# DixianZhu/deBWT

Measured on NVIDIA B200. Metric: bwt_build_throughput, higher is better.
Workload: dtype u64

## Files before the change

### debwt_b200/api.py

```python
from __future__ import annotations

import ctypes
from typing import Sequence

import numpy as np

from . import binding
from .binding import DebwtError, ShardStats, Stats, c_p, c_u64, check, lib


def _ptr(a: np.ndarray):
    return a.ctypes.data_as(c_p)


def join_records(records: Sequence) -> tuple[np.ndarray, np.ndarray]:
    arrs = [np.frombuffer(r.encode() if isinstance(r, str) else bytes(r), dtype=np.uint8)
            if not isinstance(r, np.ndarray) else r.astype(np.uint8, copy=False) for r in records]
    if not arrs:
        raise DebwtError("no records")
    n = sum(a.size for a in arrs) + len(arrs)
    text = np.empty(n, dtype=np.uint8)
    seps = np.empty(len(arrs), dtype=np.uint64)
    pos = 0
    for i, a in enumerate(arrs):
# ... 132 lines not shown
    def locate(self, patterns: Sequence) -> tuple[np.ndarray, np.ndarray]:
        pats = [p.encode() if isinstance(p, str) else bytes(p) for p in patterns]
        offs = np.zeros(len(pats) + 1, dtype=np.uint64)
        offs[1:] = np.cumsum([len(p) for p in pats])
        blob = np.frombuffer(b"".join(pats) + b"\0", dtype=np.uint8)
        hits = np.zeros(len(pats) + 1, dtype=np.uint64)
        check(lib().debwt_index_locate(self._h, _ptr(blob), _ptr(offs), len(pats), _ptr(hits), c_p(0), 0))
        pos = np.empty(int(hits[-1]), dtype=np.uint64)
        if pos.size:
            check(lib().debwt_index_locate(self._h, _ptr(blob), _ptr(offs), len(pats), _ptr(hits), _ptr(pos), pos.size))
        return hits, pos

    def verify(self, text=None, device_ptr: int | None = None, n_symbols: int | None = None):
        bad, ms = c_u64(), ctypes.c_float()
        if device_ptr is not None:
            check(lib().debwt_verify_text_device(self._h, c_p(device_ptr), n_symbols, ctypes.byref(bad), ctypes.byref(ms)))
        else:
            text = np.ascontiguousarray(text, dtype=np.uint8)
            check(lib().debwt_verify_text(self._h, _ptr(text), text.size, ctypes.byref(bad), ctypes.byref(ms)))
        return int(bad.value), float(ms.value)

    def stats(self) -> dict:
        s = Stats()
        check(lib().debwt_get_stats(self._h, ctypes.byref(s)))
        return s.as_dict()


def build_bwt(records: Sequence, device: int = 0, k: int = 32):
    with BwtBuilder(device) as b:
        b.set_records(records)
        b.build(k)
        return b.result()


def write_outputs(path: str, words: np.ndarray, sharp: np.ndarray, dollar: np.ndarray):
    words.astype("<u8", copy=False).tofile(path)
    sharp.astype("<u8", copy=False).tofile(path + ".#")
    dollar.astype("<u8", copy=False).tofile(path + ".$")


def read_outputs(path: str, n_symbols: int):
    words = np.fromfile(path, dtype="<u8").astype(np.uint64, copy=False)
    if words.size != (n_symbols + 31) // 32:
        raise DebwtError(f"{path}: {words.size} words, but {n_symbols} symbols need {(n_symbols + 31) // 32}")
    sharp = np.fromfile(path + ".#", dtype="<u8").astype(np.uint64, copy=False)
    dollar = np.fromfile(path + ".$", dtype="<u8").astype(np.uint64, copy=False)
    if dollar.size != 1:
        raise DebwtError(f"{path}.$: {dollar.size} values, expected 1")
    return words, sharp, dollar


def record_offsets(positions, seps) -> tuple[np.ndarray, np.ndarray]:
    pos = np.asarray(positions, dtype=np.uint64)
    seps = np.asarray(seps, dtype=np.uint64)
    if pos.size and int(pos.max()) > int(seps[-1]):
        raise ValueError(f"position {int(pos.max())} is beyond the text ({int(seps[-1]) + 1} symbols)")
    rec = np.searchsorted(seps, pos, side="left")
    starts = np.concatenate(([0], seps[:-1] + 1)).astype(np.uint64)
    return rec.astype(np.int64), pos - starts[rec]


def k_pack(text: np.ndarray, device: int = 0) -> np.ndarray:
    text = np.ascontiguousarray(text, dtype=np.uint8)
    out = np.empty((text.size + 32 + 31) // 32, dtype=np.uint64)
    check(lib().debwt_k_pack(device, _ptr(text), text.size, _ptr(out)))
    return out


def k_extract(text: np.ndarray, seps: np.ndarray, device: int = 0) -> np.ndarray:
    text = np.ascontiguousarray(text, dtype=np.uint8)
    seps = np.ascontiguousarray(seps, dtype=np.uint64)
    out = np.empty(text.size - 32 * seps.size, dtype=np.uint64)
    check(lib().debwt_k_extract(device, _ptr(text), text.size, _ptr(seps), seps.size, _ptr(out)))
    return out


def k_radix_sort(keys: np.ndarray, device: int = 0, cfg: int = 0):
    k = np.ascontiguousarray(keys, dtype=np.uint64).copy()
    ms = ctypes.c_float()
    check(lib().debwt_k_radix_sort_u64(device, _ptr(k), k.size, cfg, ctypes.byref(ms)))
    return k, ms.value


def k_rle(sorted_keys: np.ndarray, device: int = 0):
    s = np.ascontiguousarray(sorted_keys, dtype=np.uint64)
    km = np.empty(s.size, dtype=np.uint64)
    ct = np.empty(s.size, dtype=np.uint64)
    d = c_u64()
    check(lib().debwt_k_rle(device, _ptr(s), s.size, _ptr(km), _ptr(ct), ctypes.byref(d)))
    return km[:d.value].copy(), ct[:d.value].copy()


def k_group_masks(text: np.ndarray, seps: np.ndarray, device: int = 0) -> np.ndarray:
    text = np.ascontiguousarray(text, dtype=np.uint8)
    seps = np.ascontiguousarray(seps, dtype=np.uint64)
    out = np.empty(text.size - 32 * seps.size, dtype=np.uint16)
    check(lib().debwt_k_group_masks(device, _ptr(text), text.size, _ptr(seps), seps.size, _ptr(out)))
    return out


def bench_sort(n: int, device: int = 0, cfg: int = 0, iters: int = 5) -> float:
    ms = ctypes.c_float()
    check(lib().debwt_bench_sort(device, n, cfg, iters, ctypes.byref(ms)))
    return ms.value


def bench_sort_passes(n: int, device: int = 0, cfg: int = 0, iters: int = 5):
    ms, msp = ctypes.c_float(), ctypes.c_float()
    check(lib().debwt_bench_sort_passes(device, n, cfg, iters, ctypes.byref(ms), ctypes.byref(msp)))
    return ms.value, msp.value


def verify_bwt_device(bwt_ptr: int, n_symbols: int, sharp_rows: np.ndarray, dollar_row: int, text_ptr: int, device: int = 0):
    sharp = np.ascontiguousarray(sharp_rows, dtype=np.uint64)
    bad, ms = c_u64(), ctypes.c_float()
    check(lib().debwt_verify_bwt_device(device, c_p(bwt_ptr), n_symbols, _ptr(sharp), sharp.size, int(dollar_row), c_p(text_ptr),
                                        ctypes.byref(bad), ctypes.byref(ms)))
    return int(bad.value), float(ms.value)


def k_codes(text: np.ndarray, seps: np.ndarray, device: int = 0):
    text = np.ascontiguousarray(text, dtype=np.uint8)
    seps = np.ascontiguousarray(seps, dtype=np.uint64)
    cap = text.size + 64
    codes = np.empty(cap, dtype=np.uint8)
    head, spi, prev = np.empty(cap, dtype=np.uint64), np.empty(cap, dtype=np.uint64), np.empty(cap, dtype=np.uint8)
    nc, nb = c_u64(), c_u64()
    check(lib().debwt_k_codes(device, _ptr(text), text.size, _ptr(seps), seps.size, _ptr(codes), cap, ctypes.byref(nc), _ptr(head),
                              _ptr(spi), _ptr(prev), cap, ctypes.byref(nb)))
    return codes[:nc.value].copy(), head[:nb.value].copy(), spi[:nb.value].copy(), prev[:nb.value].copy()


def k_sort_blue(codes: np.ndarray, seg_offsets: np.ndarray, spindex: np.ndarray, prev: np.ndarray, device: int = 0):
    codes = np.ascontiguousarray(codes, dtype=np.uint8)
    offs = np.ascontiguousarray(seg_offsets, dtype=np.uint64)
    spi = np.ascontiguousarray(spindex, dtype=np.uint64).copy()
    prv = np.ascontiguousarray(prev, dtype=np.uint8).copy()
    check(lib().debwt_k_sort_blue(device, _ptr(codes), codes.size, _ptr(offs), offs.size - 1, _ptr(spi), _ptr(prv)))
    return spi, prv


def verify_walk_device(bwt_ptr: int, n_symbols: int, sharp_rows: np.ndarray, dollar_row: int, tail_ptr: int, steps: int, device: int = 0):
    sharp = np.ascontiguousarray(sharp_rows, dtype=np.uint64)
    bad = c_u64()
    carr = np.zeros(6, dtype=np.uint64)
    check(lib().debwt_verify_walk_device(device, c_p(bwt_ptr), n_symbols, _ptr(sharp), sharp.size, int(dollar_row), c_p(tail_ptr), steps,
                                         ctypes.byref(bad), _ptr(carr)))
    return int(bad.value), carr


class Shard:

    def __init__(self, device: int, rank: int, world: int, group_tag: str, same_process: bool = False, sort_config: int = 0):
        self._h = c_p()
        self.rank, self.world, self.device = rank, world, device
        check(lib().debwt_shard_create(ctypes.byref(self._h), device, rank, world, group_tag.encode(), int(same_process)))
        if sort_config:
            lib().debwt_shard_set_sort_config(self._h, sort_config)

    def close(self):
        if self._h:
            lib().debwt_shard_destroy(self._h)
            self._h = c_p()

    def __enter__(self):
        return self
# ... 59 lines not shown
```

### debwt_b200/build.py

```python
from __future__ import annotations

import concurrent.futures as cf
import os
import shutil
import subprocess

HERE = os.path.dirname(os.path.abspath(__file__))
CSRC = os.path.join(HERE, "csrc")
OBJ = os.path.join(HERE, "_build")
LIB = os.path.join(HERE, "libdebwt_b200.so")
SOURCES = ["radix_sort.cu", "radix_sort_tma.cu", "stages.cu", "bluesort.cu", "dist_kernels.cu", "dev_api.cu", "api.cu", "index.cu", "synth.cu", "shard.cu"]
HEADERS = ["common.cuh", "radix_sort.cuh", "radix_common.cuh", "ctx.cuh", "shmcomm.h", "stages.cuh", "stages_dev.cuh", "special.cuh", "dist_kernels.cuh",
           os.path.join("..", "..", "include", "debwt_b200.h"), os.path.join("..", "..", "include", "debwt_b200_dev.h")]
NVCC_FLAGS = ["-gencode", "arch=compute_100a,code=sm_100a", "-lineinfo", "-O3", "-std=c++17",
              "-Xcompiler", "-fPIC", "-Xcompiler", "-O2"]


def _nvcc() -> str:
    for cand in (shutil.which("nvcc"), "/usr/local/cuda/bin/nvcc"):
        if cand and os.path.isfile(cand):
            return cand
    raise RuntimeError("nvcc not found")


def _stale(target: str, deps) -> bool:
    if not os.path.isfile(target):
        return True
    t = os.path.getmtime(target)
    return any(os.path.getmtime(d) > t for d in deps)


def build(force: bool = False, verbose: bool = False) -> str:
    os.makedirs(OBJ, exist_ok=True)
    nvcc = _nvcc()
    hdrs = [os.path.join(CSRC, h) for h in HEADERS]
    jobs = []
    for src in SOURCES:
        s = os.path.join(CSRC, src)
        o = os.path.join(OBJ, src.replace(".cu", ".o"))
        if force or _stale(o, [s] + hdrs):
            jobs.append([nvcc] + NVCC_FLAGS + ["-c", s, "-o", o])
    if jobs:
        with cf.ThreadPoolExecutor(max_workers=len(jobs)) as ex:
            for cmd, res in zip(jobs, ex.map(lambda c: subprocess.run(c, capture_output=True, text=True), jobs)):
                if verbose or res.returncode:
                    print(" ".join(cmd))
                    print(res.stdout + res.stderr)
                if res.returncode:
                    raise RuntimeError("nvcc failed: " + " ".join(cmd))
    objs = [os.path.join(OBJ, s.replace(".cu", ".o")) for s in SOURCES]
    if force or jobs or _stale(LIB, objs):
        cmd = [nvcc, "-shared", "-o", LIB] + objs + ["-gencode", "arch=compute_100a,code=sm_100a", "-lcudart", "-lrt", "-lpthread"]
        res = subprocess.run(cmd, capture_output=True, text=True)
        if res.returncode:
            print(res.stdout + res.stderr)
            raise RuntimeError("link failed")
    return LIB


if __name__ == "__main__":
    print(build(verbose=True))
```

### debwt_b200/csrc/api.cu

```cuda
#include <algorithm>
#include <cstring>
#include <map>
#include <mutex>
#include <string>
#include <tuple>
#include <vector>

#include "../../include/debwt_b200.h"
#include "../../include/debwt_b200_dev.h"
#include "radix_sort.cuh"
#include "stages.cuh"
#include "special.cuh"
#include "ctx.cuh"
#include "dist_kernels.cuh"

namespace debwt {

static thread_local std::string g_err;
unsigned g_launches = 0;
unsigned long long g_launches_total = 0;
void set_error(const std::string& msg) { g_err = msg; }

#define FAIL(msg)            \
    do {                     \
        debwt::set_error(msg); \
        return -1;           \
    } while (0)

template <typename T>
static int dalloc(DevPool& pool, T** p, size_t count) { return pool.alloc(reinterpret_cast<void**>(p), count * sizeof(T)); }

struct Special {
    u64 pos;
    u32 j;
    u32 rec;
    u64 ins, row;
    u64 w0, w1;
    u8 chr, next;
    bool emit;
};



int build_special_tables(const SpecialInfo* info, const u64* seps, u64 R, std::vector<u64>& ins, std::vector<u64>& rows,
                         std::vector<u8>& chr, std::vector<u64>& emit_pos, std::vector<u64>& tail_pos) {
    const u64 nspec = 32 * R;
    std::vector<Special> sp(nspec);
    std::vector<char> seen_rank(nspec, 0);
    for (u64 t = 0; t < nspec; ++t) {
        const SpecialInfo& o = info[t];
        if (o.rank >= nspec || seen_rank[o.rank]) FAIL("internal: special suffix ranks are not a permutation");
        seen_rank[o.rank] = 1;
        Special& x = sp[o.rank];
        x.pos = seps[t >> 5] - (t & 31); x.j = (u32)(t & 31); x.rec = (u32)(t >> 5); x.emit = false;
        x.ins = o.ins; x.chr = o.prev; x.w0 = o.w0; x.w1 = o.w1; x.next = o.next;
    }
    ins.resize(nspec); rows.resize(nspec); chr.resize(nspec); tail_pos.assign(R, 0); emit_pos.clear();
    for (u64 t = 0; t < nspec; ++t) {
        ins[t] = sp[t].ins;
        if (t && ins[t] < ins[t - 1]) FAIL("internal: special insertion points are not monotone");
        rows[t] = ins[t] + t;
        chr[t] = sp[t].chr;
    }
    std::map<std::tuple<u32, u64, u64>, std::vector<u64>> groups;
    for (u64 t = 0; t < nspec; ++t) {
        const u32 j = sp[t].j;
        if (j == 31) { sp[t].emit = true; tail_pos[sp[t].rec] = sp[t].pos; continue; }
        if (sp[t].rec + 1 == R) continue;
        const u64 before = j ? (sp[t].w0 & ~(~0ull >> (2 * j))) : 0;
        const u64 after = sp[t].w1 & ~(~0ull >> (2 * (30 - j)));
        groups[std::make_tuple(j, before, j == 30 ? 0 : after)].push_back(t);
    }
    for (auto& g : groups) {
        if (g.second.size() < 2) continue;
        u32 seen = 0;
        for (u64 t : g.second) seen |= 1u << sp[t].next;
        if (seen & (seen - 1))
            for (u64 t : g.second) sp[t].emit = true;
    }
    for (u64 t = 0; t < nspec; ++t) if (sp[t].emit) emit_pos.push_back(sp[t].pos);
    return 0;
}

}

using namespace debwt;

namespace {

std::mutex g_pool_mutex;

int bind_device(int device) {
// ... 154 lines not shown

int debwt_set_text(debwt_ctx* c, const char* text, uint64_t n, const uint64_t* seps, uint64_t n_records) {
    if (!c || !text || !seps) FAIL("null argument");
    if (bind_device(c->device)) return -1;
    reset_input(c);
    if (check_seps(seps, n_records, n)) return -1;
    c->seps.assign(seps, seps + n_records);
    c->n = n; c->n_rec = n_records;
    c->pool.hint(n * 19 + (320ull << 20));
    CUDA_TRY(cudaEventRecord(c->ev[0], c->st));
    if (dalloc(c->pool, &c->d_ascii, n + 64)) return -1;
    CUDA_TRY(cudaMemcpyAsync(c->d_ascii, text, n, cudaMemcpyHostToDevice, c->st));
    CUDA_TRY(cudaEventRecord(c->ev[1], c->st));
    CUDA_TRY(cudaStreamSynchronize(c->st));
    CUDA_TRY(cudaEventElapsedTime(&c->stats.ms_h2d, c->ev[0], c->ev[1]));
    c->input_mark = c->pool.mark();
    return 0;
}

int debwt_set_text_device(debwt_ctx* c, const void* d_text, uint64_t n, const uint64_t* seps, uint64_t n_records) {
    if (!c || !d_text || !seps) FAIL("null argument");
    if (bind_device(c->device)) return -1;
    reset_input(c);
    if (check_seps(seps, n_records, n)) return -1;
    if (reinterpret_cast<uintptr_t>(d_text) & 15) FAIL("device text must be 16-byte aligned");
    c->seps.assign(seps, seps + n_records);
    c->n = n; c->n_rec = n_records;
    c->pool.hint(n * 18 + (320ull << 20));
    c->d_ascii_ext = reinterpret_cast<const u8*>(d_text);
    c->input_mark = c->pool.mark();
    return 0;
}

int debwt_build(debwt_ctx* c, int k) {
    if (!c) FAIL("null context");
    if (k < 12 || k > 32) FAIL("-k: k-mer length (from 12 to 32, default 32)");
    if (c->loaded) FAIL("the context holds a loaded result (debwt_set_result), not an input: set an input before building");
    if (c->n == 0) FAIL("no input set");
    if (bind_device(c->device)) return -1;
    const u8* ascii = c->d_ascii_ext ? c->d_ascii_ext : c->d_ascii;
    if (c->ing.active) FAIL("streaming input is still open: call debwt_ingest_end first");
    if (!ascii && !c->d_packed) FAIL("input was consumed by a previous build; set it again");
    cudaStream_t st = c->st;
    DevPool& pool = c->pool;
    pool.rewind(c->input_mark);
    drop_index(c);
    c->built = false;
    const u64 n = c->n, R = c->n_rec, nk = n - 32 * R;
    debwt_stats& S = c->stats;
    const float keep_h2d = S.ms_h2d;
    S = debwt_stats{};
    S.ms_h2d = keep_h2d;
    S.n_symbols = n; S.n_records = R; S.n_keys = nk; S.n_special = 32 * R;
    g_launches = 0;
    int evi = 0;
    auto mark = [&]() { cudaEventRecord(c->ev[evi++], st); };
    mark();

    u64* d_seps = nullptr; u64* d_text = nullptr; u32* d_err = nullptr;
    if (dalloc(pool, &d_seps, R)) return -1;
    CUDA_TRY(cudaMemcpyAsync(d_seps, c->seps.data(), R * 8, cudaMemcpyHostToDevice, st));
    if (c->d_packed) {
        d_text = c->d_packed;
        d_err = c->d_packed_err;
    } else {
        if (dalloc(pool, &d_text, text_words(n)) || dalloc(pool, &d_err, 4)) return -1;
        CUDA_TRY(cudaMemsetAsync(d_err, 0, 16, st));
        PackPolicy pol;
        pol.resolve = c->resolve_ambiguous; pol.seed = c->ambiguity_seed;
        if (k_pack(ascii, n, d_text, d_err, st, pol)) return -1;
        if (c->d_ascii) { pool.adopt(c->d_ascii, n + 64); c->d_ascii = nullptr; }
    }
    mark();

    u64 *d_ka = nullptr, *d_kb = nullptr;
    if (dalloc(pool, &d_ka, nk + 2) || dalloc(pool, &d_kb, nk + 2)) return -1;
    if (k_extract(d_text, n, d_seps, R, d_ka, st)) return -1;
    mark();

    void* d_sortws = nullptr;
    if (pool.alloc(&d_sortws, sort_workspace_bytes(nk, c->sort_cfg))) return -1;
    SortWorkspace ws;
    sort_workspace_bind(ws, d_sortws, nk, c->sort_cfg);
    int sweeps = 0;
    ws.ev_sweep_begin = c->ev[11]; ws.ev_sweep_end = c->ev[12]; ws.sweeps_out = &sweeps;
    const unsigned launches_before_sort = g_launches;
    u64* d_keys = nullptr;
    KeyIndex ki;
    ki.bits = key_index_bits(nk);
    if (dalloc(pool, &ki.idx, (1ull << ki.bits) + 2) || k_key_index_init(ki, st)) return -1;
    bool index_marked = false;
    ws.key_index = ki.idx; ws.key_index_bits = ki.bits; ws.key_index_done = &index_marked;
    const bool text_hist = text_digit_hist_applies(n, R);
    if (text_hist && (radix_sort_clear(ws, st) || k_text_digit_hist(d_text, n, d_seps, R, ws.hist, st))) return -1;
    if (radix_sort_u64(d_ka, d_kb, nk, ws, st, &d_keys, text_hist)) return -1;
    S.sort_launches = g_launches - launches_before_sort;
    S.sort_sweeps = (u32)sweeps;
    pool.adopt(d_keys == d_ka ? d_kb : d_ka, (nk + 2) * 8);
    pool.adopt(d_sortws, sort_workspace_bytes(nk, c->sort_cfg));
    u32 h_err[2] = {0, 0};
    CUDA_TRY(cudaMemcpyAsync(h_err, d_err, 8, cudaMemcpyDeviceToHost, st));
    mark();

    u16* d_gmask = nullptr;
    if (dalloc(pool, &d_gmask, nk + 2)) return -1;
    CUDA_TRY(cudaMemsetAsync(d_gmask, 0, (nk + 2) * 2, st));
    if (k_key_index_finish(d_keys, nk, ki, index_marked, st)) return -1;
    if (k_mark_edges(d_keys, nk, ki, d_gmask, st)) return -1;
    if (k_mark_heads_tails(d_text, d_seps, R, d_keys, nk, ki, d_gmask, st)) return -1;
    void* d_brws = nullptr; u64* d_tot = nullptr;
    if (pool.alloc(&d_brws, branch_workspace_bytes(nk)) || dalloc(pool, &d_tot, 4)) return -1;
    if (k_branch_count(d_keys, nk, d_gmask, true, d_brws, d_tot, st)) return -1;
    u64 h_tot[2] = {0, 0};
    CUDA_TRY(cudaMemcpyAsync(h_tot, d_tot, 16, cudaMemcpyDeviceToHost, st));
    CUDA_TRY(cudaStreamSynchronize(st));
    if (h_err[0]) FAIL(c->resolve_ambiguous ? "input contains a symbol that is neither a base nor an IUPAC ambiguity code"
                                            : "input contains a symbol other than A, C, G, T (either case)");
    if (h_err[1] != R) FAIL("input contains '#' or '$' inside a record (they are reserved for the record separators)");
    BranchTable bt;
    bt.n_branch = h_tot[0]; bt.n_blue = h_tot[1];
    S.n_branch = bt.n_branch; S.n_blue = bt.n_blue;
    {
        int bits = 8;
        while (bits < 27 && (1ull << bits) < 2 * bt.n_branch) ++bits;
        bt.bits = bits;
    }
    if (dalloc(pool, &bt.kmer, bt.n_branch + 1) || dalloc(pool, &bt.head, bt.n_branch + 1) ||
        dalloc(pool, &bt.blue, bt.n_branch + 2) || dalloc(pool, &bt.cursor, bt.n_branch + 1) ||
        dalloc(pool, &bt.bidx, BranchTable::index_words(bt.bits)))
        return -1;
    CUDA_TRY(cudaMemsetAsync(bt.cursor, 0, (bt.n_branch + 1) * 4, st));
    if (k_branch_write(d_keys, nk, d_gmask, d_brws, bt, st)) return -1;
    {
        const u32 m32 = (u32)bt.n_blue;
        CUDA_TRY(cudaMemcpyAsync(bt.blue + bt.n_branch, &m32, 4, cudaMemcpyHostToDevice, st));
    }
    if (k_branch_index(bt, st)) return -1;
    int id_bits = 1;
    while (id_bits < 64 && (bt.n_branch >> id_bits)) ++id_bits;
    const bool group_by_sort = id_bits <= 28 && n < (1ull << 32) && bt.n_blue > 1 &&
                               c->blue_grouping == 2;
    bt.hbits = BranchTable::hash_bits(bt.n_branch);
    bt.hmode = group_by_sort ? 0 : 1;
    if (dalloc(pool, &bt.hslots, 1ull << bt.hbits) || k_branch_hash(bt, st)) return -1;
    mark();

    const u64 nspec = 32 * R;
    std::vector<SpecialInfo> info(nspec);
    std::vector<u64> h_ins(nspec);
    u64* d_ins = nullptr;
    if (dalloc(pool, &d_ins, nspec)) return -1;
    {
        SpecialInfo* d_info = nullptr;
        if (dalloc(pool, &d_info, nspec)) return -1;
        if (k_special_scan(d_text, d_seps, R, d_keys, nk, ki, d_info, st)) return -1;
        CUDA_TRY(cudaMemcpyAsync(info.data(), d_info, nspec * sizeof(SpecialInfo), cudaMemcpyDeviceToHost, st));
        CUDA_TRY(cudaStreamSynchronize(st));
    }
    std::vector<u64> h_rows, h_emit_pos, h_tail_pos;
    std::vector<u8> h_chr;
    if (build_special_tables(info.data(), c->seps.data(), R, h_ins, h_rows, h_chr, h_emit_pos, h_tail_pos)) return -1;
    u64 *d_rows = nullptr, *d_emit = nullptr, *d_tail = nullptr, *d_tail_idx = nullptr;
    u8* d_chr = nullptr;
    if (dalloc(pool, &d_rows, nspec) || dalloc(pool, &d_chr, nspec) || dalloc(pool, &d_emit, h_emit_pos.size() + 1) ||
        dalloc(pool, &d_tail, R) || dalloc(pool, &d_tail_idx, R))
        return -1;
    CUDA_TRY(cudaMemcpyAsync(d_rows, h_rows.data(), nspec * 8, cudaMemcpyHostToDevice, st));
    CUDA_TRY(cudaMemcpyAsync(d_chr, h_chr.data(), nspec, cudaMemcpyHostToDevice, st));
    CUDA_TRY(cudaMemcpyAsync(d_ins, h_ins.data(), nspec * 8, cudaMemcpyHostToDevice, st));
    CUDA_TRY(cudaMemcpyAsync(d_emit, h_emit_pos.data(), h_emit_pos.size() * 8, cudaMemcpyHostToDevice, st));
    CUDA_TRY(cudaMemcpyAsync(d_tail, h_tail_pos.data(), R * 8, cudaMemcpyHostToDevice, st));
    mark();

    const u64 nbw = (n + 31) / 32;
    u32 *d_mo = nullptr, *d_wp = nullptr;
    u64* d_blue = nullptr;
    void* d_scanws = nullptr;
    const int id_shift = 64 - id_bits;
    u64 *d_bka = nullptr, *d_bkb = nullptr, *d_bcount = nullptr;
    void* d_bsortws = nullptr;
    const int bcfg = kDefaultSortCfg;
    if (dalloc(pool, &d_mo, nbw + 2) || dalloc(pool, &d_wp, nbw + 2) || pool.alloc(&d_scanws, scan_workspace_bytes(nbw)))
// ... 562 lines not shown
```

### debwt_b200/csrc/dev_api.cu

```cuda
#include <string.h>

#include <vector>

#include "../../include/debwt_b200_dev.h"
#include "dist_kernels.cuh"
#include "radix_sort.cuh"
#include "special.cuh"

using namespace debwt;

namespace {
inline cudaStream_t S(void* s) { return reinterpret_cast<cudaStream_t>(s); }
inline KeyIndex KI(const void* idx, int bits) {
    KeyIndex k;
    k.idx = reinterpret_cast<u32*>(const_cast<void*>(idx));
    k.bits = bits;
    return k;
}
inline BranchTable BT(const void* kmer, const void* head, const void* blue, void* cursor, const void* bidx, int bits,
                      u64 nb, u64 nblue) {
    BranchTable b;
    b.n_branch = nb; b.n_blue = nblue;
    b.kmer = reinterpret_cast<u64*>(const_cast<void*>(kmer));
    b.head = reinterpret_cast<u32*>(const_cast<void*>(head));
    b.blue = reinterpret_cast<u32*>(const_cast<void*>(blue));
    b.cursor = reinterpret_cast<u32*>(cursor);
    b.bidx = reinterpret_cast<u32*>(const_cast<void*>(bidx));
    b.bits = bits;
    return b;
}
#define P64(x) reinterpret_cast<u64*>(const_cast<void*>(static_cast<const void*>(x)))
#define P32(x) reinterpret_cast<u32*>(const_cast<void*>(static_cast<const void*>(x)))
#define P16(x) reinterpret_cast<u16*>(const_cast<void*>(static_cast<const void*>(x)))
#define P8(x) reinterpret_cast<u8*>(const_cast<void*>(static_cast<const void*>(x)))
}

extern "C" {

int debwt_dev_init(int device) {
    CUDA_TRY(cudaSetDevice(device));
    cudaMemPool_t mp;
    CUDA_TRY(cudaDeviceGetDefaultMemPool(&mp, device));
    unsigned long long thr = ~0ull;
    CUDA_TRY(cudaMemPoolSetAttribute(mp, cudaMemPoolAttrReleaseThreshold, &thr));
    return 0;
}

int debwt_dev_pack(const void* d_ascii, uint64_t n, void* d_words, uint64_t nwords, void* d_err, void* stream) {
    return k_pack_words(P8(d_ascii), n, P64(d_words), nwords, P32(d_err), S(stream));
}

int debwt_dev_extract(const void* d_words, uint64_t pos_lo, uint64_t pos_hi, const void* d_seps, uint64_t n_rec,
                      uint64_t idx_base, void* d_keys, void* stream) {
    return k_extract_range(P64(d_words), pos_lo, pos_hi, P64(d_seps), n_rec, idx_base, P64(d_keys), S(stream));
}

int debwt_dev_extract_slice(const void* d_words, uint64_t n_symbols, uint64_t pos_lo, uint64_t pos_hi, const void* d_seps,
                            uint64_t n_rec, uint64_t idx_base, void* d_keys, void* stream) {
    return k_extract_slice(P64(d_words), n_symbols, pos_lo, pos_hi, P64(d_seps), n_rec, idx_base, P64(d_keys), S(stream));
}

uint64_t debwt_dev_sort_workspace_bytes(uint64_t n, int cfg) { return sort_workspace_bytes(n, cfg); }
uint64_t debwt_dev_branch_workspace_bytes(uint64_t n) { return branch_workspace_bytes(n) + 64; }
uint64_t debwt_dev_scan_workspace_bytes(uint64_t n_words) { return scan_workspace_bytes(n_words) + 64; }

int debwt_dev_sort(void* d_a, void* d_b, uint64_t n, int cfg, void* d_workspace, int* result_in_b, void* stream) {
    SortWorkspace ws;
    sort_workspace_bind(ws, d_workspace, n, cfg);
    u64* res = nullptr;
    if (radix_sort_u64(P64(d_a), P64(d_b), n, ws, S(stream), &res)) return -1;
    if (result_in_b) *result_in_b = (res == P64(d_b)) ? 1 : 0;
    return 0;
}

int debwt_dev_sort_timed(void* d_a, void* d_b, uint64_t n, int cfg, void* d_workspace, int* result_in_b, float* ms_total,
                         float* ms_sweeps, int* n_sweeps, void* stream) {
    cudaStream_t st = S(stream);
    SortWorkspace ws;
    sort_workspace_bind(ws, d_workspace, n, cfg);
    static cudaEvent_t e[4] = {nullptr, nullptr, nullptr, nullptr};
    if (!e[0]) for (auto& x : e) CUDA_TRY(cudaEventCreate(&x));
    int sweeps = 0;
    ws.ev_sweep_begin = e[1]; ws.ev_sweep_end = e[2]; ws.sweeps_out = &sweeps;
    CUDA_TRY(cudaEventRecord(e[0], st));
    u64* res = nullptr;
    int rc = radix_sort_u64(P64(d_a), P64(d_b), n, ws, st, &res);
    CUDA_TRY(cudaEventRecord(e[3], st));
    CUDA_TRY(cudaStreamSynchronize(st));
    if (!rc) {
        if (ms_total) CUDA_TRY(cudaEventElapsedTime(ms_total, e[0], e[3]));
        if (ms_sweeps) { *ms_sweeps = 0; if (sweeps) CUDA_TRY(cudaEventElapsedTime(ms_sweeps, e[1], e[2])); }
        if (n_sweeps) *n_sweeps = sweeps;
        if (result_in_b) *result_in_b = (res == P64(d_b)) ? 1 : 0;
    }
    return rc;
}

int debwt_dev_owner_of_keys(const void* d_items, uint64_t n, const void* d_splitters, uint32_t n_split, uint64_t mask,
                            int drop_marker, void* d_dest_u8, void* stream) {
    return k_owner_of_keys(P64(d_items), n, P64(d_splitters), n_split, mask, drop_marker != 0, P8(d_dest_u8), S(stream));
}

int debwt_dev_owner_of_index(void* d_idx, uint64_t n, const void* d_bases, uint32_t n_ranks, void* d_dest_u8, void* stream) {
    return k_owner_of_index(P64(d_idx), n, P64(d_bases), n_ranks, P8(d_dest_u8), S(stream));
}

namespace {
int partition_impl(const u64* a, const u64* b, const PartitionBy& by, u64 n, u32 n_ranks, u64* out_a, u64* out_b,
                   uint64_t* counts_out, void* d_workspace, cudaStream_t st) {
    if (n_ranks == 0 || n_ranks > 16) { set_error("partition: 1..16 ranks"); return -1; }
    u64* d_counts = P64(d_workspace);
    CUDA_TRY(cudaMemsetAsync(d_counts, 0, 16 * 8, st));
    if (k_partition_count(a, by, n, n_ranks, d_counts, st)) return -1;
    u64 h[16];
    CUDA_TRY(cudaMemcpyAsync(h, d_counts, sizeof h, cudaMemcpyDeviceToHost, st));
    CUDA_TRY(cudaStreamSynchronize(st));
    u64 cur[16], run = 0;
    for (int r = 0; r < 16; ++r) { cur[r] = run; run += h[r]; if ((u32)r < n_ranks) counts_out[r] = h[r]; }
    CUDA_TRY(cudaMemcpyAsync(d_counts, cur, sizeof cur, cudaMemcpyHostToDevice, st));
    if (k_partition_scatter(a, b, by, n, n_ranks, d_counts, out_a, out_b, st)) return -1;
    CUDA_TRY(cudaStreamSynchronize(st));
    return 0;
}
}

int debwt_dev_partition(const void* d_a, const void* d_b, const void* d_dest_u8, uint64_t n, uint32_t n_ranks,
                        void* d_out_a, void* d_out_b, uint64_t* counts_out, void* d_workspace, void* stream) {
    PartitionBy by;
    by.dest = P8(d_dest_u8);
    return partition_impl(P64(d_a), d_b ? P64(d_b) : nullptr, by, n, n_ranks, P64(d_out_a), d_out_b ? P64(d_out_b) : nullptr,
                          counts_out, d_workspace, S(stream));
}

int debwt_dev_partition_by_splitters(const void* d_items, uint64_t n, const void* d_splitters, uint32_t n_split, uint64_t mask,
                                     int drop_marker, uint32_t n_ranks, void* d_out, uint64_t* counts_out, void* d_workspace,
                                     void* stream) {
    PartitionBy by;
    by.splitters = P64(d_splitters); by.n_split = n_split; by.mask = mask; by.drop_marker = drop_marker != 0;
    return partition_impl(P64(d_items), nullptr, by, n, n_ranks, P64(d_out), nullptr, counts_out, d_workspace, S(stream));
}

int debwt_dev_ipc_alloc(uint64_t bytes, void** d_ptr, unsigned char handle_out[64]) {
    static_assert(sizeof(cudaIpcMemHandle_t) == 64, "IPC handle size is part of the ABI");
    CUDA_TRY(cudaMalloc(d_ptr, bytes ? bytes : 256));
    cudaIpcMemHandle_t h;
    CUDA_TRY(cudaIpcGetMemHandle(&h, *d_ptr));
    memcpy(handle_out, &h, 64);
    return 0;
}

int debwt_dev_ipc_open(const unsigned char handle[64], void** d_ptr) {
    cudaIpcMemHandle_t h;
    memcpy(&h, handle, 64);
    CUDA_TRY(cudaIpcOpenMemHandle(d_ptr, h, cudaIpcMemLazyEnablePeerAccess));
    return 0;
}

int debwt_dev_ipc_close(void* d_ptr) {
    CUDA_TRY(cudaIpcCloseMemHandle(d_ptr));
    return 0;
}

int debwt_dev_ipc_free(void* d_ptr) {
    CUDA_TRY(cudaFree(d_ptr));
    return 0;
}

int debwt_dev_partition_count(const void* d_items, uint64_t n, const void* d_splitters, uint32_t n_split, uint64_t mask,
                              int drop_marker, uint32_t n_ranks, uint64_t* counts_out, void* d_workspace, void* stream) {
    if (n_ranks == 0 || n_ranks > 16) { set_error("partition: 1..16 ranks"); return -1; }
    cudaStream_t st = S(stream);
    PartitionBy by;
    by.splitters = P64(d_splitters); by.n_split = n_split; by.mask = mask; by.drop_marker = drop_marker != 0;
    u64* d_counts = P64(d_workspace);
    CUDA_TRY(cudaMemsetAsync(d_counts, 0, 16 * 8, st));
    if (k_partition_count(P64(d_items), by, n, n_ranks, d_counts, st)) return -1;
    u64 h[16];
    CUDA_TRY(cudaMemcpyAsync(h, d_counts, sizeof h, cudaMemcpyDeviceToHost, st));
    CUDA_TRY(cudaStreamSynchronize(st));
    for (u32 r = 0; r < n_ranks; ++r) counts_out[r] = h[r];
// ... 153 lines not shown
```

### include/debwt_b200_dev.h

```cpp
#ifndef DEBWT_B200_DEV_H
#define DEBWT_B200_DEV_H

#include <stdint.h>

#ifdef __cplusplus
extern "C" {
#endif

int debwt_dev_init(int device);

int debwt_dev_pack(const void* d_ascii, uint64_t n, void* d_words, uint64_t nwords, void* d_err, void* stream);
int debwt_dev_extract(const void* d_words, uint64_t pos_lo, uint64_t pos_hi, const void* d_seps, uint64_t n_rec,
                      uint64_t idx_base, void* d_keys, void* stream);
int debwt_dev_extract_slice(const void* d_words, uint64_t n_symbols, uint64_t pos_lo, uint64_t pos_hi, const void* d_seps,
                            uint64_t n_rec, uint64_t idx_base, void* d_keys, void* stream);
uint64_t debwt_dev_sort_workspace_bytes(uint64_t n, int cfg);
uint64_t debwt_dev_branch_workspace_bytes(uint64_t n);
uint64_t debwt_dev_scan_workspace_bytes(uint64_t n_words);
int debwt_dev_sort(void* d_a, void* d_b, uint64_t n, int cfg, void* d_workspace, int* result_in_b, void* stream);
int debwt_dev_sort_timed(void* d_a, void* d_b, uint64_t n, int cfg, void* d_workspace, int* result_in_b, float* ms_total,
                         float* ms_sweeps, int* n_sweeps, void* stream);
int debwt_dev_owner_of_keys(const void* d_items, uint64_t n, const void* d_splitters, uint32_t n_split, uint64_t mask,
                            int drop_marker, void* d_dest_u8, void* stream);
int debwt_dev_owner_of_index(void* d_idx, uint64_t n, const void* d_bases, uint32_t n_ranks, void* d_dest_u8, void* stream);
int debwt_dev_partition(const void* d_a, const void* d_b, const void* d_dest_u8, uint64_t n, uint32_t n_ranks,
                        void* d_out_a, void* d_out_b, uint64_t* counts_out, void* d_workspace, void* stream);
int debwt_dev_partition_by_splitters(const void* d_items, uint64_t n, const void* d_splitters, uint32_t n_split, uint64_t mask,
                                     int drop_marker, uint32_t n_ranks, void* d_out, uint64_t* counts_out, void* d_workspace,
                                     void* stream);
int debwt_dev_ipc_alloc(uint64_t bytes, void** d_ptr, unsigned char handle_out[64]);
int debwt_dev_ipc_open(const unsigned char handle[64], void** d_ptr);
int debwt_dev_ipc_close(void* d_ptr);
int debwt_dev_ipc_free(void* d_ptr);
int debwt_dev_partition_count(const void* d_items, uint64_t n, const void* d_splitters, uint32_t n_split, uint64_t mask,
                              int drop_marker, uint32_t n_ranks, uint64_t* counts_out, void* d_workspace, void* stream);
int debwt_dev_partition_scatter_p2p(const void* d_items, uint64_t n, const void* d_splitters, uint32_t n_split, uint64_t mask,
                                    int drop_marker, uint32_t n_ranks, void* const* dst, void* d_workspace, void* stream);
int debwt_dev_key_index_bits(uint64_t n);
int debwt_dev_key_index(const void* d_sorted, uint64_t n, void* d_idx_u32, int bits, void* stream);
int debwt_dev_out_edges_queries(const void* d_sorted, uint64_t n, void* d_gmask, void* d_queries, void* stream);
int debwt_dev_apply_in_queries(const void* d_sorted, uint64_t n, const void* d_idx_u32, int bits, void* d_gmask,
                               const void* d_queries, uint64_t m, void* stream);
int debwt_dev_heads_tails(const void* d_words, const void* d_seps, uint64_t n_rec, const void* d_sorted, uint64_t n,
                          const void* d_idx_u32, int bits, void* d_gmask, void* stream);
int debwt_dev_propagate(const void* d_sorted, uint64_t n, void* d_gmask, void* stream);
int debwt_dev_branch_count(const void* d_sorted, uint64_t n, const void* d_gmask, uint64_t* n_branch, uint64_t* n_blue,
                           void* d_workspace, void* stream);
int debwt_dev_branch_write(const void* d_sorted, uint64_t n, const void* d_gmask, void* workspace, void* d_kmer,
                           void* d_head_u32, void* d_blue_u32 , uint64_t n_branch, uint64_t n_blue, void* stream);
uint64_t debwt_dev_branch_index_words(int bits);
int debwt_dev_branch_index(const void* d_kmer, uint64_t n_branch, void* d_bidx_u32, int bits, void* stream);
int debwt_dev_special_scan(const void* d_words, const void* d_seps, uint64_t n_rec, const void* d_sorted, uint64_t n,
                           const void* d_idx_u32, int bits, void* d_info, void* stream);
int debwt_special_tables(const void* info_host, const uint64_t* ins_by_t, const uint64_t* seps, uint64_t n_rec,
                         uint64_t* ins_out, uint64_t* rows_out, uint8_t* chr_out, uint64_t* emit_pos_out,
                         uint64_t* n_emit_out, uint64_t* tail_pos_out);
int debwt_dev_flag_slice(const void* d_words, uint64_t pos_lo, uint64_t pos_hi, const void* d_seps, uint64_t n_rec,
                         const void* d_gkmer, uint64_t n_branch_total, const void* d_bidx_u32, int bits, void* d_mo_bits,
                         void* d_rec_entry, void* d_rec_index, void* d_rec_count, void* stream);
int debwt_dev_patch_bits_slice(void* d_mo_bits, uint64_t pos_lo, uint64_t pos_hi, const void* d_positions, uint64_t m,
                               void* stream);
int debwt_dev_scan_popc(const void* d_mo_bits, void* d_word_prefix, uint64_t nbw, uint64_t* total, void* d_workspace,
                        void* stream);
int debwt_dev_emit_codes_slice(const void* d_words, uint64_t word_lo, uint64_t nbw, const void* d_mo_bits,
                               const void* d_word_prefix, uint64_t code_base, void* d_codes, void* stream);
int debwt_dev_mark_sep_slice(const void* d_mo_bits, const void* d_word_prefix, uint64_t pos_lo, uint64_t pos_hi,
                             uint64_t code_base, const void* d_positions, uint64_t m, void* d_sep, void* d_out_idx,
                             void* stream);
int debwt_dev_fix_records(void* d_rec_entry, uint64_t m, const void* d_mo_bits, const void* d_word_prefix, uint64_t pos_lo,
                          uint64_t code_base, void* stream);
int debwt_dev_scatter_blue(const void* d_rec_entry, const void* d_rec_local, uint64_t m, const void* d_kmer,
                           const void* d_blue_u32, void* d_cursor_u32, uint64_t n_branch, void* d_blue, void* stream);
int debwt_dev_sort_blue(void* d_blue, const void* d_kmer, const void* d_blue_u32, uint64_t n_branch, uint64_t n_blue,
                        const void* d_codes, const void* d_sep, uint64_t dollar_index, uint64_t n_codes, void* d_work_u32,
                        void* stream);
int debwt_dev_fill_range(const void* d_gmask, uint64_t n_keys, uint64_t key_base, uint64_t n_symbols,
                         const void* d_spec_rows, uint64_t m, uint64_t word_lo, uint64_t word_hi, void* d_bwt, void* stream);
int debwt_dev_emit_blue(const void* d_blue, const void* d_kmer, const void* d_head_u32, const void* d_blue_u32,
                        uint64_t n_branch, uint64_t n_blue, uint64_t key_base, const void* d_spec_ins, uint64_t m,
                        void* d_bwt, void* d_sharp_rows, void* d_sharp_count_u32, void* d_dollar_row, void* stream);
int debwt_dev_emit_special(const void* d_spec_rows, const void* d_spec_chr, uint64_t m, void* d_bwt, void* stream);

#ifdef __cplusplus
}
#endif
#endif
```

Measured before the change: 9058.

## Replace full LSD radix sort with MSD bucket pass plus in-shared-memory bucket sort

Sorts k-mer keys by first running the radix sort only on the top 16/24 bits to bucket them, then sorting each group of small buckets entirely in shared memory, skipping digits that do not vary, and building the key index there. Oversized buckets are gathered and radix-sorted separately, or the code falls back to a full radix sort when too many keys land in big buckets. This aims to cut the global-memory passes of a full 8-pass LSD sort. In exchange it adds a host synchronization to read the big-bucket totals and a dependence on a reasonably uniform key distribution.

After: 9074, median of 6. Within noise of the previous version (+0.2%).

```diff
diff --git a/debwt_b200/api.py b/debwt_b200/api.py
--- a/debwt_b200/api.py
+++ b/debwt_b200/api.py
@@ -238,6 +238,28 @@
     return k, ms.value
 
 
+def dev_kmer_sort(keys, cfg: int = 8, timed: bool = False):
+    import torch
+    n = keys.numel()
+    L = lib()
+    L.debwt_dev_kmer_sort_workspace_bytes.restype = c_u64
+    L.debwt_dev_kmer_sort_workspace_bytes.argtypes = [c_u64, ctypes.c_int]
+    ws = torch.empty(int(L.debwt_dev_kmer_sort_workspace_bytes(n, cfg)), dtype=torch.uint8, device=keys.device)
+    tmp = torch.empty_like(keys)
+    st = ctypes.c_void_p(torch.cuda.current_stream(keys.device).cuda_stream)
+    in_b = ctypes.c_int(0)
+    args = [ctypes.c_void_p(keys.data_ptr()), ctypes.c_void_p(tmp.data_ptr()), c_u64(n), ctypes.c_int(cfg),
+            ctypes.c_void_p(ws.data_ptr()), ctypes.byref(in_b)]
+    if not timed:
+        check(L.debwt_dev_kmer_sort(*args, st))
+        return tmp if in_b.value else keys
+    ms = (ctypes.c_float * 4)()
+    sweeps, big = ctypes.c_int(), c_u64()
+    check(L.debwt_dev_kmer_sort_timed(*args, ms, ctypes.byref(sweeps), ctypes.byref(big), st))
+    stats = {"ms": ms[0], "ms_top": ms[1], "ms_buckets": ms[2], "ms_big": ms[3], "sweeps": sweeps.value, "big_keys": big.value}
+    return (tmp if in_b.value else keys), stats
+
+
 def k_rle(sorted_keys: np.ndarray, device: int = 0):
     s = np.ascontiguousarray(sorted_keys, dtype=np.uint64)
     km = np.empty(s.size, dtype=np.uint64)
diff --git a/debwt_b200/build.py b/debwt_b200/build.py
--- a/debwt_b200/build.py
+++ b/debwt_b200/build.py
@@ -9,8 +9,8 @@
 CSRC = os.path.join(HERE, "csrc")
 OBJ = os.path.join(HERE, "_build")
 LIB = os.path.join(HERE, "libdebwt_b200.so")
-SOURCES = ["radix_sort.cu", "radix_sort_tma.cu", "stages.cu", "bluesort.cu", "dist_kernels.cu", "dev_api.cu", "api.cu", "index.cu", "synth.cu", "shard.cu"]
-HEADERS = ["common.cuh", "radix_sort.cuh", "radix_common.cuh", "ctx.cuh", "shmcomm.h", "stages.cuh", "stages_dev.cuh", "special.cuh", "dist_kernels.cuh",
+SOURCES = ["radix_sort.cu", "bucket_sort.cu", "radix_sort_tma.cu", "stages.cu", "bluesort.cu", "dist_kernels.cu", "dev_api.cu", "api.cu", "index.cu", "synth.cu", "shard.cu"]
+HEADERS = ["common.cuh", "radix_sort.cuh", "bucket_sort.cuh", "radix_common.cuh", "ctx.cuh", "shmcomm.h", "stages.cuh", "stages_dev.cuh", "special.cuh", "dist_kernels.cuh",
            os.path.join("..", "..", "include", "debwt_b200.h"), os.path.join("..", "..", "include", "debwt_b200_dev.h")]
 NVCC_FLAGS = ["-gencode", "arch=compute_100a,code=sm_100a", "-lineinfo", "-O3", "-std=c++17",
               "-Xcompiler", "-fPIC", "-Xcompiler", "-O2"]
diff --git a/debwt_b200/csrc/api.cu b/debwt_b200/csrc/api.cu
--- a/debwt_b200/csrc/api.cu
+++ b/debwt_b200/csrc/api.cu
@@ -8,6 +8,7 @@
 
 #include "../../include/debwt_b200.h"
 #include "../../include/debwt_b200_dev.h"
+#include "bucket_sort.cuh"
 #include "radix_sort.cuh"
 #include "stages.cuh"
 #include "special.cuh"
@@ -328,22 +329,25 @@
     if (pool.alloc(&d_sortws, sort_workspace_bytes(nk, c->sort_cfg))) return -1;
     SortWorkspace ws;
     sort_workspace_bind(ws, d_sortws, nk, c->sort_cfg);
-    int sweeps = 0;
-    ws.ev_sweep_begin = c->ev[11]; ws.ev_sweep_end = c->ev[12]; ws.sweeps_out = &sweeps;
+    ws.ev_sweep_begin = c->ev[11]; ws.ev_sweep_end = c->ev[12];
     const unsigned launches_before_sort = g_launches;
-    u64* d_keys = nullptr;
     KeyIndex ki;
     ki.bits = key_index_bits(nk);
     if (dalloc(pool, &ki.idx, (1ull << ki.bits) + 2) || k_key_index_init(ki, st)) return -1;
-    bool index_marked = false;
-    ws.key_index = ki.idx; ws.key_index_bits = ki.bits; ws.key_index_done = &index_marked;
+    const size_t kws_bytes = kmer_sort_workspace_bytes(nk, ki.bits);
+    void* d_kws = nullptr;
+    if (kws_bytes && pool.alloc(&d_kws, kws_bytes)) return -1;
     const bool text_hist = text_digit_hist_applies(n, R);
     if (text_hist && (radix_sort_clear(ws, st) || k_text_digit_hist(d_text, n, d_seps, R, ws.hist, st))) return -1;
-    if (radix_sort_u64(d_ka, d_kb, nk, ws, st, &d_keys, text_hist)) return -1;
+    KmerSortResult ks;
+    if (kmer_sort(d_ka, d_kb, nk, ws, d_kws, ki, text_hist, st, &ks)) return -1;
+    u64* d_keys = ks.keys;
+    const bool index_marked = ks.index_marked;
     S.sort_launches = g_launches - launches_before_sort;
-    S.sort_sweeps = (u32)sweeps;
+    S.sort_sweeps = (u32)ks.sweeps;
     pool.adopt(d_keys == d_ka ? d_kb : d_ka, (nk + 2) * 8);
     pool.adopt(d_sortws, sort_workspace_bytes(nk, c->sort_cfg));
+    if (kws_bytes) pool.adopt(d_kws, kws_bytes);
     u32 h_err[2] = {0, 0};
     CUDA_TRY(cudaMemcpyAsync(h_err, d_err, 8, cudaMemcpyDeviceToHost, st));
     mark();
diff --git a/debwt_b200/csrc/bucket_sort.cu b/debwt_b200/csrc/bucket_sort.cu
--- /dev/null
+++ b/debwt_b200/csrc/bucket_sort.cu
@@ -0,0 +1,260 @@
+#include "bucket_sort.cuh"
+#include "radix_common.cuh"
+
+namespace debwt {
+
+namespace {
+
+using namespace radix;
+
+constexpr int BS_THREADS = 256;
+constexpr int BS_ITEMS = 16;
+constexpr int BS_WARPS = BS_THREADS / 32;
+constexpr u32 BS_CAP = BS_THREADS * BS_ITEMS;
+constexpr u32 BS_SLICE = BS_CAP - BS_CAP / 8;
+constexpr u64 KMER_SORT_MIN_KEYS = 1ull << 19;
+
+struct BigBucket { u32 start, len, off, bucket; };
+
+__global__ void __launch_bounds__(BS_THREADS, 3)
+bucket_sort_kernel(u64* keys, u32 n, const u32* __restrict__ tab, int bbits, u32* __restrict__ kidx, int kshift,
+                   BigBucket* __restrict__ big, u32* __restrict__ big_totals ) {
+    __shared__ __align__(16) u64 s_keys[BS_CAP];
+    __shared__ u32 s_whist[BS_WARPS * RADIX];
+    __shared__ u32 s_scan[40];
+    __shared__ u64 s_or, s_and;
+    __shared__ u32 s_seg[4];
+    const int tid = threadIdx.x, lane = tid & 31, warp = tid >> 5;
+    const int bshift = 64 - bbits;
+    const u32 nb = 1u << bbits;
+    const u32 lo = blockIdx.x * BS_SLICE;
+    const u32 hi = min(lo + BS_SLICE, n);
+    u32 c = 0, E = 0, bc = 0, b_hi = 0;
+    if (tid == 0) {
+        u32 b = (u32)(keys[lo] >> bshift);
+        if (tab[b] < lo) ++b;
+        bc = b;
+        c = tab[b];
+        if (hi == n) {
+            b_hi = nb;
+        } else {
+            b_hi = (u32)(keys[hi] >> bshift);
+            if (tab[b_hi] < hi) ++b_hi;
+        }
+        E = tab[b_hi];
+    }
+    const u32 lt = lanemask_lt();
+    u32* wh = s_whist + warp * RADIX;
+    for (;;) {
+        if (tid == 0) {
+            u32 len = 0;
+            if (c >= E) {
+                s_seg[3] = 1;
+            } else {
+                s_seg[3] = 0;
+                u32 p = bc + 1;
+                if (E - c <= BS_CAP) {
+                    p = b_hi;
+                    len = E - c;
+                } else if (tab[p] - c > BS_CAP) {
+                    const u32 l = tab[p] - c;
+                    const u32 slot = atomicAdd(big_totals, 1u);
+                    big[slot] = BigBucket{c, l, atomicAdd(big_totals + 1, l), bc};
+                } else {
+                    while (p < b_hi && tab[p + 1] - c <= BS_CAP) ++p;
+                    len = tab[p] - c;
+                }
+                s_seg[0] = c;
+                s_seg[1] = len;
+                c = tab[p];
+                bc = p;
+            }
+            s_or = 0;
+            s_and = ~0ull;
+        }
+        __syncthreads();
+        if (s_seg[3]) break;
+        const u32 base = s_seg[0], len = s_seg[1];
+        if (len == 0) { __syncthreads(); continue; }
+        for (u32 i = tid; i < BS_CAP; i += BS_THREADS) s_keys[i] = i < len ? keys[base + i] : ~0ull;
+        __syncthreads();
+        u64 key[BS_ITEMS];
+        const u32 first = warp * (BS_ITEMS * 32) + lane;
+        u64 vor = 0, vand = ~0ull;
+#pragma unroll
+        for (int j = 0; j < BS_ITEMS; ++j) {
+            key[j] = s_keys[first + j * 32];
+            if (first + j * 32 < len) { vor |= key[j]; vand &= key[j]; }
+        }
+#pragma unroll
+        for (int o = 16; o; o >>= 1) {
+            vor |= __shfl_xor_sync(0xffffffffu, vor, o);
+            vand &= __shfl_xor_sync(0xffffffffu, vand, o);
+        }
+        if (lane == 0) { atomicOr(&s_or, vor); atomicAnd(&s_and, vand); }
+        __syncthreads();
+        const u64 vary = s_or ^ s_and;
+        int last = -1;
+        for (int d = 0; d < PASSES; ++d) if ((vary >> (8 * d)) & 255u) last = d;
+        for (int d = 0; d <= last; ++d) {
+            if (!((vary >> (8 * d)) & 255u)) continue;
+            const int sh = 8 * d;
+            for (int i = tid; i < BS_WARPS * RADIX; i += BS_THREADS) s_whist[i] = 0;
+            __syncthreads();
+            u32 rank2[BS_ITEMS / 2];
+#pragma unroll
+            for (int j = 0; j < BS_ITEMS; ++j) {
+                const u32 dg = (u32)(key[j] >> sh) & 255u;
+                const u32 peers = match_digit(dg);
+                const u32 below = __popc(peers & lt);
+                const u32 pre = wh[dg];
+                __syncwarp();
+                if (below == 0) wh[dg] = pre + __popc(peers);
+                __syncwarp();
+                const u32 r = pre + below;
+                if (j & 1) rank2[j >> 1] |= r << 16; else rank2[j >> 1] = r;
+            }
+            __syncthreads();
+            u32 part = 0;
+#pragma unroll
+            for (int w = 0; w < BS_WARPS; ++w) {
+                const u32 v = s_whist[w * RADIX + tid];
+                s_whist[w * RADIX + tid] = part;
+                part += v;
+            }
+            const u32 off = block_exclusive_scan<BS_THREADS>(part, nullptr, s_scan);
+#pragma unroll
+            for (int w = 0; w < BS_WARPS; ++w) s_whist[w * RADIX + tid] += off;
+            __syncthreads();
+#pragma unroll
+            for (int j = 0; j < BS_ITEMS; ++j) {
+                const u32 dg = (u32)(key[j] >> sh) & 255u;
+                const u32 r = (j & 1) ? (rank2[j >> 1] >> 16) : (rank2[j >> 1] & 0xffffu);
+                s_keys[wh[dg] + r] = key[j];
+            }
+            __syncthreads();
+            if (d != last) {
+#pragma unroll
+                for (int j = 0; j < BS_ITEMS; ++j) key[j] = s_keys[first + j * 32];
+            }
+        }
+        for (u32 i = tid; i < len; i += BS_THREADS) {
+            const u64 k = s_keys[i];
+            if (last >= 0) keys[base + i] = k;
+            if (i == 0 || (s_keys[i - 1] >> kshift) != (k >> kshift)) kidx[k >> kshift] = base + i;
+        }
+        __syncthreads();
+    }
+}
+
+__global__ void __launch_bounds__(256) big_gather_kernel(const u64* __restrict__ keys, const BigBucket* __restrict__ big,
+                                                         u64* __restrict__ out) {
+    const BigBucket e = big[blockIdx.x];
+    for (u32 i = threadIdx.x; i < e.len; i += 256) out[e.off + i] = keys[e.start + i];
+}
+
+__global__ void __launch_bounds__(256) big_return_kernel(u64* __restrict__ keys, const BigBucket* __restrict__ big,
+                                                         const u64* __restrict__ sorted, u32 m, int bbits, u32* __restrict__ kidx,
+                                                         int kshift) {
+    __shared__ u32 s_from;
+    const BigBucket e = big[blockIdx.x];
+    if (threadIdx.x == 0) s_from = (u32)lower_bound_u64(sorted, 0, m, (u64)e.bucket << (64 - bbits));
+    __syncthreads();
+    const u64* src = sorted + s_from;
+    for (u32 i = threadIdx.x; i < e.len; i += 256) {
+        const u64 k = src[i];
+        keys[e.start + i] = k;
+        if (i == 0 || (src[i - 1] >> kshift) != (k >> kshift)) kidx[k >> kshift] = e.start + i;
+    }
+}
+
+}
+
+int kmer_sort_bucket_bits(u64 n, int key_index_bits) {
+    if (n < KMER_SORT_MIN_KEYS || n >= (1ull << 32) - (1u << 16)) return 0;
+    return key_index_bits >= 24 ? 24 : 16;
+}
+
+size_t kmer_sort_workspace_bytes(u64 n, int key_index_bits) {
+    const int bb = kmer_sort_bucket_bits(n, key_index_bits);
+    if (!bb) return 0;
+    return (((1ull << bb) + 1) * 4 + 255) / 256 * 256 + (n / (BS_CAP + 1) + 1) * sizeof(BigBucket) + 64;
+}
+
+int kmer_sort(u64* a, u64* b, u64 n, const SortWorkspace& ws, void* workspace, KeyIndex ki, bool hist_ready, cudaStream_t st,
+              KmerSortResult* res) {
+    res->keys = a;
+    res->sweeps = 0;
+    res->index_marked = false;
+    res->big_buckets = res->big_keys = 0;
+    const int bb = kmer_sort_bucket_bits(n, ki.bits);
+    if (!bb) {
+        SortWorkspace w = ws;
+        w.key_index = ki.idx; w.key_index_bits = ki.bits; w.key_index_done = &res->index_marked; w.sweeps_out = &res->sweeps;
+        w.first_pass = 0;
+        if (res->ev[0]) CUDA_TRY(cudaEventRecord(res->ev[0], st));
+        if (radix_sort_u64(a, b, n, w, st, &res->keys, hist_ready)) return -1;
+        for (int i = 1; i < 4; ++i) if (res->ev[i]) CUDA_TRY(cudaEventRecord(res->ev[i], st));
+        return 0;
+    }
+    char* p = static_cast<char*>(workspace);
+    KeyIndex tab;
+    tab.idx = reinterpret_cast<u32*>(p);
+    tab.bits = bb;
+    p += (((1ull << bb) + 1) * 4 + 255) / 256 * 256;
+    u32* totals = reinterpret_cast<u32*>(p);
+    BigBucket* big = reinterpret_cast<BigBucket*>(p + 64);
+
+    if (res->ev[0]) CUDA_TRY(cudaEventRecord(res->ev[0], st));
+    if (k_key_index_init(tab, st)) return -1;
+    CUDA_TRY(cudaMemsetAsync(totals, 0, 8, st));
+    bool tab_marked = false;
+    SortWorkspace w = ws;
+    w.key_index = tab.idx; w.key_index_bits = bb; w.key_index_done = &tab_marked; w.sweeps_out = &res->sweeps;
+    w.first_pass = PASSES - bb / 8;
+    u64* keys = nullptr;
+    if (radix_sort_u64(a, b, n, w, st, &keys, hist_ready)) return -1;
+    u64* other = keys == a ? b : a;
+    if (k_key_index_finish(keys, n, tab, tab_marked, st)) return -1;
+    if (res->ev[1]) CUDA_TRY(cudaEventRecord(res->ev[1], st));
+
+    const int kshift = 64 - ki.bits;
+    const u64 slices = (n + BS_SLICE - 1) / BS_SLICE;
+    bucket_sort_kernel<<<(unsigned)slices, BS_THREADS, 0, st>>>(keys, (u32)n, tab.idx, bb, ki.idx, kshift, big, totals);
+    CUDA_TRY(cudaGetLastError());
+    DEBWT_COUNT(1);
+    u32 h_tot[2] = {0, 0};
+    CUDA_TRY(cudaMemcpyAsync(h_tot, totals, 8, cudaMemcpyDeviceToHost, st));
+    if (res->ev[2]) CUDA_TRY(cudaEventRecord(res->ev[2], st));
+    CUDA_TRY(cudaStreamSynchronize(st));
+    res->big_buckets = h_tot[0];
+    res->big_keys = h_tot[1];
+    res->keys = keys;
+    res->index_marked = true;
+
+    const u64 m = h_tot[1], half = (n / 2) & ~1ull;
+    if (m > half) {
+        if (k_key_index_init(ki, st)) return -1;
+        SortWorkspace f = ws;
+        f.ev_sweep_begin = f.ev_sweep_end = nullptr;
+        int more = 0;
+        f.key_index = ki.idx; f.key_index_bits = ki.bits; f.key_index_done = &res->index_marked; f.sweeps_out = &more;
+        f.first_pass = 0;
+        if (radix_sort_u64(keys, other, n, f, st, &res->keys)) return -1;
+        res->sweeps += more;
+    } else if (m) {
+        big_gather_kernel<<<h_tot[0], 256, 0, st>>>(keys, big, other);
+        CUDA_TRY(cudaGetLastError());
+        SortWorkspace f;
+        sort_workspace_bind(f, ws.hist, m, ws.cfg);
+        u64* sorted = nullptr;
+        if (radix_sort_u64(other, other + half, m, f, st, &sorted)) return -1;
+        big_return_kernel<<<h_tot[0], 256, 0, st>>>(keys, big, sorted, (u32)m, bb, ki.idx, kshift);
+        CUDA_TRY(cudaGetLastError());
+        DEBWT_COUNT(2);
+    }
+    if (res->ev[3]) CUDA_TRY(cudaEventRecord(res->ev[3], st));
+    return 0;
+}
+
+}
diff --git a/debwt_b200/csrc/bucket_sort.cuh b/debwt_b200/csrc/bucket_sort.cuh
--- /dev/null
+++ b/debwt_b200/csrc/bucket_sort.cuh
@@ -0,0 +1,21 @@
+#pragma once
+#include "radix_sort.cuh"
+#include "stages.cuh"
+
+namespace debwt {
+
+struct KmerSortResult {
+    cudaEvent_t ev[4] = {nullptr, nullptr, nullptr, nullptr};
+    u64* keys = nullptr;
+    int sweeps = 0;
+    bool index_marked = false;
+    u64 big_buckets = 0;
+    u64 big_keys = 0;
+};
+
+int kmer_sort_bucket_bits(u64 n, int key_index_bits);
+size_t kmer_sort_workspace_bytes(u64 n, int key_index_bits);
+int kmer_sort(u64* a, u64* b, u64 n, const SortWorkspace& ws, void* workspace, KeyIndex ki, bool hist_ready, cudaStream_t st,
+              KmerSortResult* res);
+
+}
diff --git a/debwt_b200/csrc/dev_api.cu b/debwt_b200/csrc/dev_api.cu
--- a/debwt_b200/csrc/dev_api.cu
+++ b/debwt_b200/csrc/dev_api.cu
@@ -3,6 +3,7 @@
 #include <vector>
 
 #include "../../include/debwt_b200_dev.h"
+#include "bucket_sort.cuh"
 #include "dist_kernels.cuh"
 #include "radix_sort.cuh"
 #include "special.cuh"
@@ -96,6 +97,56 @@
     return rc;
 }
 
+namespace {
+inline u64 ws_align(u64 b) { return (b + 255) & ~255ull; }
+
+int kmer_sort_dev(void* d_a, void* d_b, uint64_t n, int cfg, void* d_workspace, KmerSortResult* res, cudaStream_t st) {
+    char* p = static_cast<char*>(d_workspace);
+    SortWorkspace ws;
+    sort_workspace_bind(ws, p, n, cfg);
+    p += ws_align(sort_workspace_bytes(n, cfg));
+    KeyIndex ki;
+    ki.bits = key_index_bits(n);
+    void* kws = p;
+    p += ws_align(kmer_sort_workspace_bytes(n, ki.bits));
+    ki.idx = reinterpret_cast<u32*>(p);
+    if (k_key_index_init(ki, st)) return -1;
+    return kmer_sort(P64(d_a), P64(d_b), n, ws, kws, ki, false, st, res);
+}
+}
+
+uint64_t debwt_dev_kmer_sort_workspace_bytes(uint64_t n, int cfg) {
+    const int kb = key_index_bits(n);
+    return ws_align(sort_workspace_bytes(n, cfg)) + ws_align(kmer_sort_workspace_bytes(n, kb)) + ((1ull << kb) + 2) * 4;
+}
+
+int debwt_dev_kmer_sort(void* d_a, void* d_b, uint64_t n, int cfg, void* d_workspace, int* result_in_b, void* stream) {
+    KmerSortResult res;
+    if (kmer_sort_dev(d_a, d_b, n, cfg, d_workspace, &res, S(stream))) return -1;
+    if (result_in_b) *result_in_b = (res.keys == P64(d_b)) ? 1 : 0;
+    return 0;
+}
+
+int debwt_dev_kmer_sort_timed(void* d_a, void* d_b, uint64_t n, int cfg, void* d_workspace, int* result_in_b, float* ms_phases,
+                              int* n_sweeps, uint64_t* big_keys, void* stream) {
+    cudaStream_t st = S(stream);
+    static cudaEvent_t e[4] = {nullptr, nullptr, nullptr, nullptr};
+    if (!e[0]) for (auto& x : e) CUDA_TRY(cudaEventCreate(&x));
+    KmerSortResult res;
+    for (int i = 0; i < 4; ++i) res.ev[i] = e[i];
+    int rc = kmer_sort_dev(d_a, d_b, n, cfg, d_workspace, &res, st);
+    CUDA_TRY(cudaStreamSynchronize(st));
+    if (rc) return rc;
+    if (ms_phases) {
+        CUDA_TRY(cudaEventElapsedTime(ms_phases + 0, e[0], e[3]));
+        for (int i = 0; i < 3; ++i) CUDA_TRY(cudaEventElapsedTime(ms_phases + 1 + i, e[i], e[i + 1]));
+    }
+    if (n_sweeps) *n_sweeps = res.sweeps;
+    if (big_keys) *big_keys = res.big_keys;
+    if (result_in_b) *result_in_b = (res.keys == P64(d_b)) ? 1 : 0;
+    return 0;
+}
+
 int debwt_dev_owner_of_keys(const void* d_items, uint64_t n, const void* d_splitters, uint32_t n_split, uint64_t mask,
                             int drop_marker, void* d_dest_u8, void* stream) {
     return k_owner_of_keys(P64(d_items), n, P64(d_splitters), n_split, mask, drop_marker != 0, P8(d_dest_u8), S(stream));
diff --git a/include/debwt_b200_dev.h b/include/debwt_b200_dev.h
--- a/include/debwt_b200_dev.h
+++ b/include/debwt_b200_dev.h
@@ -20,6 +20,10 @@
 int debwt_dev_sort(void* d_a, void* d_b, uint64_t n, int cfg, void* d_workspace, int* result_in_b, void* stream);
 int debwt_dev_sort_timed(void* d_a, void* d_b, uint64_t n, int cfg, void* d_workspace, int* result_in_b, float* ms_total,
                          float* ms_sweeps, int* n_sweeps, void* stream);
+uint64_t debwt_dev_kmer_sort_workspace_bytes(uint64_t n, int cfg);
+int debwt_dev_kmer_sort(void* d_a, void* d_b, uint64_t n, int cfg, void* d_workspace, int* result_in_b, void* stream);
+int debwt_dev_kmer_sort_timed(void* d_a, void* d_b, uint64_t n, int cfg, void* d_workspace, int* result_in_b, float* ms_phases,
+                              int* n_sweeps, uint64_t* big_keys, void* stream);
 int debwt_dev_owner_of_keys(const void* d_items, uint64_t n, const void* d_splitters, uint32_t n_split, uint64_t mask,
                             int drop_marker, void* d_dest_u8, void* stream);
 int debwt_dev_owner_of_index(void* d_idx, uint64_t n, const void* d_bases, uint32_t n_ranks, void* d_dest_u8, void* stream);
```
